# kasvii/GATOR

Hardware: AMD Instinct MI355X
Metric: meshes/sec (B=256, J=17) GATOR forward (higher is better)
Workload: dtype f32; 1 GPU; B=256 synthetic Human3.6M 17-joint poses per GPU, GAT+MDR forward fp32; batch_per_gpu=256, global_batch=256, num_joint=17, impl=fused, parallelism=dp1, mode=gather

## Files before the change

gator_amd/csrc/forward_plan.h:

```cpp
#pragma once
#include <cstddef>

#ifdef __HIP__
#define GATOR_PLAN_HD __host__ __device__
#else
#define GATOR_PLAN_HD
#endif

namespace gator {

constexpr int kVT = 14;
constexpr int kMdrCtrChunks = 64;
constexpr int kTiledTokens = 128;

struct FusedOptions {
    bool gat_x3 = true;
    bool gat8 = true;
    bool gat8_h4 = true;
    bool gat8_lobyte = true;
    bool gat8_tail = true;
    bool gat_tiled_h4 = true;
    int gat_tiled = -1;
    int gat_tiled_min_batch = 1024;
    int mdr_x3 = 2;
    int up_x3 = 2;
    int mdr_persist = -1;
    int mdr_persist_chunk = 0;
    int mdr_persist_grid = 0;
    bool mdr_head_partials = true;
    bool c3_mdr = true;
    bool c3_encoder = true;
    bool c3_up_w1 = true;
    bool c3_up_bf16 = false;
    bool c3_guard = true;
    bool graph = false;
    int subbatch_streams = 0;
    int gat8_dbg = 0;
    bool gat_stamps = false;
    int mdr_cut = 0;
    bool mdr_stamps = false;
    bool mdr_solo = false;
    bool mdr_ends = false;
};

constexpr int kCtrError = 8, kCtrDone = 32;
struct MdrChunkPlan {
    int nch, base, rem;
    GATOR_PLAN_HD void locate(int b, int& ch, int& b0, int& n) const {
        const int split = rem * (base + 1);
        if (b < split) { ch = b / (base + 1); n = base + 1; b0 = ch * n; }
        else { ch = rem + (b - split) / base; n = base; b0 = split + (ch - rem) * base; }
    }
    GATOR_PLAN_HD size_t block(int ch) const {
        const int big = ch < rem ? ch : rem;
        return (size_t)ch * kCtrDone + 4 * ((size_t)big * (base + 1) + (size_t)(ch - big) * base);
    }
};
inline bool operator==(const MdrChunkPlan& a, const MdrChunkPlan& b) { return a.nch == b.nch && a.base == b.base && a.rem == b.rem; }

struct Gat8Form { bool h4; int lr; bool h2, lb, tail; };
struct GatForm { bool x3k, tail; };
struct TiledForm { int J; bool h4, h2; };
inline bool operator==(const Gat8Form& a, const Gat8Form& b) { return a.h4 == b.h4 && a.lr == b.lr && a.h2 == b.h2 && a.lb == b.lb && a.tail == b.tail; }
inline bool operator==(const GatForm& a, const GatForm& b) { return a.x3k == b.x3k && a.tail == b.tail; }
inline bool operator==(const TiledForm& a, const TiledForm& b) { return a.J == b.J && a.h4 == b.h4 && a.h2 == b.h2; }
enum class PlanEntry { FORWARD, GAT, MDR };
enum class SampleEncoder { NONE, GAT, GAT8 };
enum class CtrZero { NOBODY, MDR_JOINT, GAT_JOINT, GAT8_TAIL };
enum class MdrHead { FINISH, WHOLE_HOIST, WHOLE };
enum class Regressor { NONE, FP32, X3, X2, BF16 };
struct RegressorPlan { Regressor form; bool with_joints, w1; };

struct ForwardPlan {
    int n_tiled = 0, n_tail = 0;
    SampleEncoder sample = SampleEncoder::NONE;
    TiledForm tiled{0, false, false};
    Gat8Form gat8{false, 0, false, false, false};
    GatForm gat{false, false};
    bool enc16 = false, fused_tail = false;
    CtrZero ctr_zero = CtrZero::NOBODY;
    int xa = -1, grid = 0; bool persist = false;
    MdrChunkPlan chunks{1, 0, 0};
    MdrHead head = MdrHead::FINISH; RegressorPlan up{Regressor::NONE, false, false};
};
inline bool operator==(const ForwardPlan& a, const ForwardPlan& b) {
    return a.n_tiled == b.n_tiled && a.n_tail == b.n_tail && a.sample == b.sample && a.tiled == b.tiled && a.gat8 == b.gat8 && a.gat == b.gat && a.enc16 == b.enc16 &&
           a.fused_tail == b.fused_tail && a.ctr_zero == b.ctr_zero && a.xa == b.xa && a.grid == b.grid && a.persist == b.persist && a.chunks == b.chunks &&
           a.head == b.head && a.up.form == b.up.form && a.up.with_joints == b.up.with_joints && a.up.w1 == b.up.w1;
}

inline int plan_tiled_samples(const FusedOptions& o, int J, int n_cu, int B, int pin) {
    if (!o.gat_x3 || pin == 0) return 0;
    if (pin == 1) return B;
    if (B < o.gat_tiled_min_batch) return 0;
    const int round = n_cu * (kTiledTokens / J), n_tiled = (B / round) * round;
    return B - n_tiled > 4 * n_cu ? B : n_tiled;
}

inline RegressorPlan plan_regressor(const FusedOptions& o, bool bf16, bool with_joints) {
    const Regressor form = bf16 && o.c3_up_bf16 ? Regressor::BF16 : o.up_x3 == 0 ? Regressor::FP32 : o.up_x3 == 2 ? Regressor::X2 : Regressor::X3;
    return RegressorPlan{form, with_joints, form == Regressor::X2 && bf16 && o.c3_up_w1};
}

inline bool plan_mdr_persist(const FusedOptions& o, int n_cu, int B) {
    if (o.mdr_stamps) return false;
    if (o.mdr_persist >= 0) return o.mdr_persist > 0;
    return n_cu == 256 && (B * kVT + 3) / 4 >= 3 * n_cu;
}

inline MdrChunkPlan plan_mdr_chunks(const FusedOptions& o, int xa, int B) {
    int nch = o.mdr_persist_chunk > 0 ? (B + o.mdr_persist_chunk - 1) / o.mdr_persist_chunk : (xa == 3 ? (B + 383) / 384 : B / 256);
    nch = nch < 1 ? 1 : nch > kMdrCtrChunks ? kMdrCtrChunks : nch;
    return MdrChunkPlan{nch, B / nch, B % nch};
}

inline const char* plan_forward(const FusedOptions& o, int J, int n_cu, int B, PlanEntry entry, bool bf16, bool with_joints, int pin, ForwardPlan* out) {
    ForwardPlan p;
    if (with_joints && (o.up_x3 == 0 || bf16)) return "gator_forward_joints_f32 needs the split-precision vertex regressor";
    if (entry == PlanEntry::GAT) {
        p.sample = SampleEncoder::GAT; p.gat = GatForm{o.gat_x3, true};
        *out = p;
        return nullptr;
    }
    if (entry == PlanEntry::FORWARD) {
        p.n_tiled = plan_tiled_samples(o, J, n_cu, B, pin);
        p.enc16 = bf16 && o.c3_encoder;
        if (p.n_tiled > 0 && p.enc16 && !o.gat_tiled_h4) return "the 16-bit encoder needs the four-product weight image (GATOR_GAT_TILED_H4=1, the default)";
        if (p.n_tiled > 0) p.tiled = TiledForm{J == 17 ? 17 : 19, o.gat_tiled_h4, p.enc16};
        if (p.n_tiled < B && !o.gat8) {
            p.sample = SampleEncoder::GAT; p.gat = GatForm{o.gat_x3, false};
        } else if (p.n_tiled < B) {
            p.sample = SampleEncoder::GAT8;
            if (p.enc16 && !o.gat8_h4) return "the 16-bit encoder needs the four-product weight stream (GATOR_GAT8_H4=1, the default)";
            if (J > 20) return "k_gat8: more than 20 joints (gator_create admits 17 and 19)";
            const bool lb = o.gat8_lobyte && !p.enc16;
            p.fused_tail = o.gat8_tail && (p.enc16 || o.gat8_lobyte);
            if (p.fused_tail && !(o.gat8_h4 && (p.enc16 || lb))) return "k_gat8: no fused tail on the three-plane weight stream";
            p.gat8 = o.gat8_h4 ? Gat8Form{true, J <= 18 ? 10 : 12, p.enc16, lb, p.fused_tail} : Gat8Form{false, 16, false, false, false};
        }
        p.n_tail = p.fused_tail ? p.n_tiled : B;
    }
    if (o.mdr_persist != 0) p.ctr_zero = entry == PlanEntry::MDR ? CtrZero::MDR_JOINT : p.fused_tail ? CtrZero::GAT8_TAIL : CtrZero::GAT_JOINT;
    const bool half16 = bf16 && o.c3_mdr;
    if (half16 && o.mdr_x3 != 2) return "16-bit MDR layers need GATOR_MDR_X3=2 (the default)";
    p.xa = half16 ? 3 : o.mdr_x3;
    p.persist = plan_mdr_persist(o, n_cu, B);
    p.grid = !p.persist ? 0 : o.mdr_persist_grid > 0 ? o.mdr_persist_grid : 2 * n_cu;
    p.chunks = p.persist ? plan_mdr_chunks(o, p.xa, B) : MdrChunkPlan{1, B, 0};
    p.head = o.mdr_head_partials ? MdrHead::FINISH : B <= 2 * n_cu ? MdrHead::WHOLE_HOIST : MdrHead::WHOLE;
    p.up = plan_regressor(o, bf16, with_joints);
    *out = p;
    return nullptr;
}

}
```

gator_amd/csrc/fused_api.hip:

```cpp
#include <hip/hip_runtime.h>

#include <algorithm>
#include <cmath>
#include <cstdlib>
#include <type_traits>
#include <vector>

#include "fused_state.h"
#include "x3_common.h"

namespace gator {
namespace {

static void graph_slot_free(FusedState::GraphSlot& g) {
    if (g.exec) (void)hipGraphExecDestroy((hipGraphExec_t)g.exec);
    if (g.graph) (void)hipGraphDestroy((hipGraph_t)g.graph);
    g.exec = g.graph = nullptr;
}
static void graphs_clear(FusedState* f) {
    for (auto& g : f->graphs) graph_slot_free(g);
    f->graphs.clear();
}
int fused_ensure_ws(gator_ctx* c, FusedWs& w, int B) {
    FusedState* f = c->fused;
    if (w.base && B <= w.cap) return GATOR_OK;
    if (w.base) {
        GATOR_HIP_CHECK(hipDeviceSynchronize());
        graphs_clear(f);
    }
    const int cap = B, MT = (cap + 31) / 32, J = c->J;
    const size_t tiles = (size_t)cap * kVT * 2 * kTile;
    size_t n = 0;
    auto layout = [&](float* block) {
        n = 0;
        auto region = [&](auto*& member, size_t floats) {
            if (block) member = reinterpret_cast<std::remove_reference_t<decltype(member)>>(block + n);
            n += (floats + 63) & ~(size_t)63;
        };
        region(w.vcp, (size_t)MT * 3 * kCB * kTile); region(w.vc, (size_t)cap * kV * 3);
        region(w.vf, 3 * tiles); region(w.q, 9 * tiles / 2); region(w.k, 9 * tiles / 2); region(w.v, 9 * tiles / 2);
        region(w.jkv, (size_t)cap * 12 * kTile); region(w.hf, (size_t)cap * kV * 32); region(w.lbf, (size_t)cap * kV * kE);
        region(w.feat, (size_t)cap * J * kC); region(w.vcp3, std::max(upsample_x3_vcp_elems(cap), upsample_x2_vcp_elems(cap)) / 2);
        region(w.lpart, gat_tail_part_floats(cap, J)); region(w.mdr_ctr, mdr_ctr_words(cap)); region(w.hpart, (size_t)cap * kVT * 128);
    };
    layout(nullptr);
    GATOR_TRY(w.base.alloc(n * sizeof(float)));
    GATOR_HIP_CHECK(hipMemset(w.base, 0, n * sizeof(float)));
    GATOR_HIP_CHECK(hipDeviceSynchronize());
    w.cap = cap;
    layout(w.base);
    return GATOR_OK;
}

std::vector<float> d2h(const float* p, size_t n) {
    std::vector<float> v(n);
    (void)hipMemcpy(v.data(), p, n * sizeof(float), hipMemcpyDeviceToHost);
    return v;
}

template <class F>
void fill_tile(float* dst, F tab) {
    for (int g = 0; g < 4; ++g)
        for (int lane = 0; lane < 64; ++lane)
            for (int j = 0; j < 4; ++j) dst[(g * 64 + lane) * 4 + j] = tab(lane & 31, 8 * g + 4 * (lane >> 5) + j);
}

int read_fused_options(const gator_ctx* c, FusedOptions* o) {
    auto flag = [](const char* name, bool dflt) { const char* e = getenv(name); return e ? atoi(e) != 0 : dflt; };
    auto num = [](const char* name, int dflt) { const char* e = getenv(name); return e ? atoi(e) : dflt; };
    auto set = [](const char* name) { return getenv(name) != nullptr; };
    const bool exact = c->arithmetic == GATOR_ARITH_EXACT_SPLIT;
    o->gat_x3 = flag("GATOR_GAT_X3", true);
    o->gat8 = o->gat_x3 && flag("GATOR_GAT8", true);
    o->gat8_h4 = !exact && flag("GATOR_GAT8_H4", true);
    o->gat8_lobyte = o->gat8 && o->gat8_h4 && flag("GATOR_GAT8_LOBYTE", true);
    o->gat_tiled_h4 = !exact && flag("GATOR_GAT_TILED_H4", true);
    o->gat_tiled = num("GATOR_GAT_TILED", -1);
    if (const int m = num("GATOR_GAT_TILED_MIN_BATCH", 0); m > 0) o->gat_tiled_min_batch = m;
    o->mdr_x3 = exact ? 1 : num("GATOR_MDR_X3", 2);
    o->up_x3 = exact ? 1 : num("GATOR_UPSAMPLE_X3", 2);
    if (c->parts & GATOR_PART_MDR) {
        if (o->up_x3 < 0 || o->up_x3 > 2) return fail(GATOR_EINVAL, "GATOR_UPSAMPLE_X3 must be 0, 1 or 2");
        if (o->mdr_x3 < 0 || o->mdr_x3 > 2) return fail(GATOR_EINVAL, "GATOR_MDR_X3 must be 0, 1 or 2");
    }
    o->gat8_tail = o->gat8 && o->gat8_h4 && o->mdr_x3 == 2 && flag("GATOR_GAT8_TAIL", true);
    o->mdr_persist = set("GATOR_MDR_PERSIST") ? flag("GATOR_MDR_PERSIST", false) : -1;
    o->mdr_persist_chunk = num("GATOR_MDR_PERSIST_CHUNK", 0);
    o->mdr_persist_grid = num("GATOR_MDR_PERSIST_GRID", 0);
    o->mdr_head_partials = flag("GATOR_MDR_HEAD_PARTIALS", true);
    o->c3_mdr = o->mdr_x3 == 2 && flag("GATOR_C3_MDR", true);
    o->c3_encoder = o->gat8 && o->gat8_h4 && o->gat_tiled_h4 && flag("GATOR_C3_ENCODER", true);
    o->c3_up_w1 = flag("GATOR_C3_UPSAMPLE_W1", true);
    o->c3_up_bf16 = o->up_x3 != 2 || flag("GATOR_C3_UPSAMPLE_BF16", false);
    o->c3_guard = flag("GATOR_C3_GUARD", true);
    o->graph = flag("GATOR_GRAPH", false);
    o->subbatch_streams = num("GATOR_SUBBATCH_STREAMS", 0);
#ifdef GATOR_DIAG
    o->gat8_dbg = num("GATOR_GAT8_DBG", 0);
    o->gat_stamps = set("GATOR_GAT_STAMPS");
    o->mdr_cut = num("GATOR_MDR_CUT", 0);
    o->mdr_stamps = set("GATOR_MDR_STAMPS");
    o->mdr_solo = set("GATOR_MDR_SOLO");
    o->mdr_ends = set("GATOR_MDR_ENDS");
#endif
    return GATOR_OK;
}

static double sym_eig_max(std::vector<double>& A, int n) {
    for (int sweep = 0; sweep < 64; ++sweep) {
        double off = 0, all = 0;
        for (int p = 0; p < n; ++p)
            for (int q = 0; q < n; ++q) { all += A[p * n + q] * A[p * n + q]; if (q > p) off += A[p * n + q] * A[p * n + q]; }
        if (!(off > 1e-30 * all)) break;
        for (int p = 0; p < n; ++p)
            for (int q = p + 1; q < n; ++q) {
                const double apq = A[p * n + q];
                if (apq == 0) continue;
                const double th = (A[q * n + q] - A[p * n + p]) / (2 * apq);
                const double t = (th >= 0 ? 1.0 : -1.0) / (std::fabs(th) + std::sqrt(th * th + 1));
                const double cs = 1 / std::sqrt(t * t + 1), sn = t * cs;
                for (int k = 0; k < n; ++k) {
                    const double kp = A[k * n + p], kq = A[k * n + q];
                    A[k * n + p] = cs * kp - sn * kq; A[k * n + q] = sn * kp + cs * kq;
                }
                for (int k = 0; k < n; ++k) {
                    const double pk = A[p * n + k], qk = A[q * n + k];
                    A[p * n + k] = cs * pk - sn * qk; A[q * n + k] = sn * pk + cs * qk;
                }
            }
    }
    double m = 0;
    for (int i = 0; i < n; ++i) m = std::max(m, A[i * n + i]);
    return m;
}

static double sigma_max_rows(const std::vector<float>& W, int r0, int n, int K) {
    std::vector<double> G((size_t)n * n);
    for (int i = 0; i < n; ++i)
        for (int j = 0; j < n; ++j) {
            double acc = 0;
            for (int k = 0; k < K; ++k) acc += (double)W[(size_t)(r0 + i) * K + k] * (double)W[(size_t)(r0 + j) * K + k];
            G[i * n + j] = acc;
        }
    return std::sqrt(std::max(sym_eig_max(G, n), 0.0));
}
static double norm_rows(const std::vector<float>& v, int r0, int n) {
    double s = 0;
    for (int i = 0; i < n; ++i) s += (double)v[r0 + i] * v[r0 + i];
    return std::sqrt(s);
}
static double max_abs(const std::vector<float>& v) {
    double m = 0;
    for (float x : v) m = std::max(m, (double)std::fabs(x));
    return m;
}

float c3_logit_bound(const Weights& w, const float* hop_bias, int J) {
    double worst = 0;
    for (int li = 0; li < 3; ++li) {
        const MdrLayerW& r = w.lay[li];
        const std::vector<float> wq = d2h(r.sa_w[0], 64 * 64), wk = d2h(r.sa_w[1], 64 * 64), bq = d2h(r.sa_b[0], 64), bk = d2h(r.sa_b[1], 64),
                                 a2 = d2h(r.a2, 64), b2 = d2h(r.b2, 64);
        const double xn = max_abs(a2) * std::sqrt(63.0) + norm_rows(b2, 0, 64);
        for (int hd = 0; hd < 2; ++hd)
            worst = std::max(worst, (sigma_max_rows(wq, 32 * hd, 32, 64) * xn + norm_rows(bq, 32 * hd, 32)) *
                                        (sigma_max_rows(wk, 32 * hd, 32, 64) * xn + norm_rows(bk, 32 * hd, 32)) / std::sqrt(32.0));
        const std::vector<float> cq = d2h(r.wq, 64 * 64), ck = d2h(r.wk, 64 * 64), n1w = d2h(r.n1w, 64), n1b = d2h(r.n1b, 64);
// ... 232 lines not shown
                if (rc) return rc;
                if (!h3_set_holds(ratio)) h3_demote(f, GATOR_H3SET_MDR);
            }
            if (f->opt.mdr_x3 != 2) rc = fused_repack_x3(f->lay[0].wq, f->wxbuf, ntiles, stream);
            if (rc) return rc;
        }
        float* hbd = take(64);
        GATOR_HIP_CHECK(hipMemcpy(hbd, hb.data(), 32 * sizeof(float), hipMemcpyHostToDevice));
        f->head_b = hbd;
    }
    {
        float* dst = take(10 * kTile);
        int rc = fused_pack_linear(w.jfeat_w, 133, 1, 64, 133, dst, stream);
        if (rc) return rc;
        f->jfeat_p = dst;
        float* d128 = take(8 * kTile);
        rc = fused_pack_linear(w.jfeat_w + 5, 133, 1, 64, 128, d128, stream);
        if (rc) return rc;
        f->jfeat128_p = d128;
        if (f->opt.mdr_x3 == 2) {
            float& ratio = f->h3_tile_ratio[GATOR_H3SET_JFEAT];
            GATOR_TRY(f->jf128_h3.alloc((size_t)8 * kTileX3 * sizeof(float)));
            rc = fused_repack_h3(d128, f->jf128_h3, 8, &f->jf128_wshift, &ratio, stream);
            if (rc) return rc;
            if (!h3_set_holds(ratio)) { f->jf128_h3.reset(); h3_demote(f, GATOR_H3SET_JFEAT); }
        }
        const std::vector<float> jw = d2h(w.jfeat_w, 64 * 133);
        std::vector<float> j5(5 * 64);
        for (int i = 0; i < 5; ++i)
            for (int n = 0; n < 64; ++n) j5[i * 64 + n] = jw[n * 133 + i];
        float* j5d = take(kTile);
        GATOR_HIP_CHECK(hipMemcpy(j5d, j5.data(), j5.size() * sizeof(float), hipMemcpyHostToDevice));
        f->jfeat5 = j5d;
        const std::vector<float> pj = d2h(w.pos_j, (size_t)(c->J + 1) * 64);
        std::vector<float> pt(2 * kTile);
        for (int nb = 0; nb < 2; ++nb)
            fill_tile(pt.data() + (size_t)nb * kTile, [&](int t, int ch) { return t < c->J ? pj[(size_t)(t + 1) * 64 + 32 * nb + ch] : 0.f; });
        float* pd = take(2 * kTile);
        GATOR_HIP_CHECK(hipMemcpy(pd, pt.data(), pt.size() * sizeof(float), hipMemcpyHostToDevice));
        f->posj_T = pd;
    }
    {
        const std::vector<float> vw = d2h(w.vfeat_w, 64 * 6), vb = d2h(w.vfeat_b, 64), pv = d2h(w.pos_v, (size_t)(kV + 1) * 64), v4 = d2h(w.v431, kV * 3);
        std::vector<float> base((size_t)kVT * 2 * kTile, 0.f), w3(3 * 64);
        for (int t = 0; t < kVT; ++t)
            for (int nb = 0; nb < 2; ++nb)
                for (int g = 0; g < 4; ++g)
                    for (int lane = 0; lane < 64; ++lane)
                        for (int j = 0; j < 4; ++j) {
                            const int token = 32 * t + (lane & 31), ch = 32 * nb + 8 * g + 4 * (lane >> 5) + j;
                            if (token >= kV) continue;
                            double s = (double)vb[ch];
                            for (int i = 0; i < 3; ++i) s += (double)vw[ch * 6 + i] * (double)v4[token * 3 + i];
                            base[(((size_t)(t * 2 + nb) * 4 + g) * 64 + lane) * 4 + j] = (float)(s + (double)pv[(size_t)(token + 1) * 64 + ch]);
                        }
        for (int i = 0; i < 3; ++i)
            for (int ch = 0; ch < 64; ++ch) w3[i * 64 + ch] = vw[ch * 6 + 3 + i];
        float* bd = take(base.size());
        GATOR_HIP_CHECK(hipMemcpy(bd, base.data(), base.size() * sizeof(float), hipMemcpyHostToDevice));
        f->tok_base = bd;
        float* wd = take(3 * 64);
        GATOR_HIP_CHECK(hipMemcpy(wd, w3.data(), w3.size() * sizeof(float), hipMemcpyHostToDevice));
        f->tok_w3 = wd;
    }
    GATOR_HIP_CHECK(hipStreamSynchronize((hipStream_t)stream));
    return GATOR_OK;
}

FusedState::~FusedState() {
    for (FusedWs& w : sets) { w.base.reset(); w.vcp16.reset(); }
    graphs_clear(this);
    if (cap_stream) (void)hipStreamDestroy((hipStream_t)cap_stream);
    if (aux_stream) (void)hipStreamDestroy((hipStream_t)aux_stream);
    if (ev_fork) (void)hipEventDestroy((hipEvent_t)ev_fork);
    if (ev_join) (void)hipEventDestroy((hipEvent_t)ev_join);
}

void fused_destroy(gator_ctx* c) {
    delete c->fused;
    c->fused = nullptr;
}

int launch_upsample_any(const FusedState* f, const gator_ctx* c, const FusedWs& ws, const RegressorPlan& r, int B, float* verts, void* stream) {
    return r.form == Regressor::FP32 ? launch_upsample(f, c, ws, B, verts, stream) : r.form == Regressor::X2 ? launch_upsample_x2(f, c, ws, B, verts, stream, r.with_joints, r.w1) : launch_upsample_x3(f, c, ws, B, verts, stream, r.with_joints);
}

static int fused_plan(const gator_ctx* c, int B, PlanEntry entry, bool bf16, bool with_joints, ForwardPlan* p) {
    const FusedState* f = c->fused;
    const char* why = plan_forward(f->opt, c->J, f->n_cu, B, entry, bf16, with_joints, f->gat_tiled, p);
    return why ? fail(GATOR_EUNSUPPORTED, "%s", why) : GATOR_OK;
}

int fused_gat_forward(gator_ctx* c, const float* pose2d, int B, float* x_out, float* feat, void* stream) {
    ForwardPlan p;
    GATOR_TRY(fused_plan(c, B, PlanEntry::GAT, false, false, &p));
    StageTimer tm(c, "gat", stream);
    return launch_gat(c, c->fused, p.gat, pose2d, B, x_out, feat, stream, B, 0);
}

int fused_upsample(gator_ctx* c, const float* vert431, int B, float* verts, void* stream) {
    FusedState* f = c->fused;
    FusedWs& ws = f->sets[0];
    GATOR_TRY(fused_ensure_ws(c, ws, B));
    const RegressorPlan r = plan_regressor(f->opt, false, false);
    int rc = r.form == Regressor::FP32 ? launch_pack_vc(vert431, B, ws.vcp, stream)
         : r.form == Regressor::X2 ? launch_pack_vc_x2(vert431, B, ws.vcp3, stream) : launch_pack_vc_x3(vert431, B, ws.cap, ws.vcp3, stream);
    if (rc) return rc;
    StageTimer tm(c, "upsample", stream);
    return launch_upsample_any(f, c, ws, r, B, verts, stream);
}

static int fused_upsample_bf16_in(gator_ctx* c, FusedWs& ws, const float* vert431, int B, float* verts, void* stream) {
    GATOR_TRY(fused_ensure_ws(c, ws, B));
    FusedState* f = c->fused;
    if (!f->up_w16) {
        GATOR_TRY(f->up_w16.alloc(upsample_bf16_weight_elems() * 2));
        GATOR_TRY(pack_upsample_bf16(c->w.up_w, f->up_w16, stream));
        GATOR_HIP_CHECK(hipStreamSynchronize((hipStream_t)stream));
    }
    if (B > ws.vcp16_cap) {
        if (ws.vcp16) GATOR_HIP_CHECK(hipDeviceSynchronize());
        GATOR_TRY(ws.vcp16.alloc(upsample_bf16_vcp_elems(B) * 2));
        ws.vcp16_cap = B;
    }
    StageTimer tm(c, "upsample_bf16", stream);
    return launch_upsample_bf16(f, c, ws, vert431, B, verts, stream);
}

int fused_upsample_bf16(gator_ctx* c, const float* vert431, int B, float* verts, void* stream) {
    return fused_upsample_bf16_in(c, c->fused->sets[0], vert431, B, verts, stream);
}

static int fused_regress(gator_ctx* c, FusedWs& ws, const RegressorPlan& r, int B, float* verts, void* stream) {
    if (r.form == Regressor::BF16) return fused_upsample_bf16_in(c, ws, ws.vc, B, verts, stream);
    StageTimer tm(c, "upsample", stream);
    return launch_upsample_any(c->fused, c, ws, r, B, verts, stream);
}

int fused_mdr_forward(gator_ctx* c, const float* pc, int B, float* verts, void* stream) {
    FusedWs& ws = c->fused->sets[0];
    ForwardPlan p;
    GATOR_TRY(fused_plan(c, B, PlanEntry::MDR, false, false, &p));
    GATOR_TRY(fused_ensure_ws(c, ws, B));
    GATOR_TRY(launch_mdr(c, c->fused, ws, p, pc, B, stream, nullptr, nullptr));
    return fused_regress(c, ws, p.up, B, verts, stream);
}

static int fused_forward_one(gator_ctx* c, FusedWs& ws, const ForwardPlan& p, const float* pose2d, int B, float* verts, float* pose3d, void* stream, float* joints);

int fused_set_graph_replay(gator_ctx* c, int on) {
    FusedState* f = c->fused;
    if (!f) return fail(GATOR_EUNSUPPORTED, "gator_set_graph_replay: fused ctx only");
    if (on >= 0) {
        if (!on && f->graph_replay) { GATOR_HIP_CHECK(hipDeviceSynchronize()); graphs_clear(f); }
        f->graph_replay = on != 0;
    }
    return (int)std::min<unsigned long long>(f->graph_launches, 0x7fffffffull);
}

static int fused_forward_graph(gator_ctx* c, FusedWs& ws, const ForwardPlan& p, const float* pose2d, int B, float* verts, float* pose3d, void* stream) {
    FusedState* f = c->fused;
    int rc = fused_ensure_ws(c, ws, B);
    if (rc) return rc;
    FusedState::GraphSlot* slot = nullptr;
    for (auto& g : f->graphs)
        if (g.B == B && g.in == pose2d && g.verts == verts && g.pose3d == pose3d && g.ws == ws.base.get() && g.plan == p) { slot = &g; break; }
    if (!slot) {
        if ((int)f->graphs.size() >= FusedState::kGraphSlots) {
            auto lru = std::min_element(f->graphs.begin(), f->graphs.end(), [](const FusedState::GraphSlot& a, const FusedState::GraphSlot& b) {
                return (a.exec != nullptr) != (b.exec != nullptr) ? a.exec == nullptr : a.used < b.used; });
            if (lru->exec) GATOR_HIP_CHECK(hipDeviceSynchronize());
            graph_slot_free(*lru);
            f->graphs.erase(lru);
        }
        FusedState::GraphSlot g;
        g.B = B; g.in = pose2d; g.verts = verts; g.pose3d = pose3d; g.plan = p; g.ws = ws.base.get();
        g.used = ++f->graph_clock;
        f->graphs.push_back(g);
        return fused_forward_one(c, ws, p, pose2d, B, verts, pose3d, stream, nullptr);
    }
    slot->used = ++f->graph_clock;
    if (!slot->exec) {
        if (!f->cap_stream) {
            hipStream_t s2;
            GATOR_HIP_CHECK(hipStreamCreateWithFlags(&s2, hipStreamNonBlocking));
            f->cap_stream = s2;
        }
// ... 174 lines not shown
```

gator_amd/csrc/fused_state.h:

```cpp
#pragma once
#include "internal.h"
#include "forward_plan.h"
#include <vector>

namespace gator {

constexpr int kOB = 216;
constexpr int kCB = 14;
constexpr int kTile = 32 * 32;
__host__ __device__ inline size_t mdr_ctr_words(int B) { return (size_t)32 * kMdrCtrChunks + (size_t)4 * B; }

struct MdrLayerP {
    const float *wq, *wk, *wv, *proj, *fc1, *fc2, *sa[4];
};

enum { V_N1W = 0, V_N1B = 128, V_QKVB = 256, V_PROJB = 640, V_GCNB = 768, V_LIN0B = 896, V_BACKB = 1024, V_N2W = 1152,
       V_N2B = 1280, V_FC1B = 1408, V_FC2B = 1920, V_TOTAL = 2048 };

struct GatBlockPk {
    const float *qkv, *proj, *w0, *w1, *lin0, *lin1, *back, *fc1, *fc2;
    const float *mc, *mdT, *aoffT, *f1b;
};

struct FusedWs {
// ... 35 lines not shown
    DevBuf<float> jf128_h3;
    int jf128_wshift = 0;
    int mdr_wshift = 0;
    float h3_tile_ratio[4] = {0.f, 0.f, 0.f, 0.f};
    int h3_demoted = 0;
    float c3_logit_bound = 0.f;
    DevBuf<void> up_w2;
    float up_w2_unscale = 1.f;
    DevBuf<void> up_w16;
    DevBuf<void> jr_blk, jr_ent;
    DevBuf<float> jr_w;
    DevBuf<int> jr_rowptr;
    DevBuf<float> jr_P;
    int jr_nnz = 0, jr_nj = 0, jr_cap = 0;
    DevBuf<float> blk_tap;
    int blk_tap_cap = 0;
    MdrLayerP lay[3];
    const float* head_w = nullptr;
    const float* head_b = nullptr;
    const float* tok_base = nullptr;
    const float* tok_w3 = nullptr;
    struct GraphSlot {
        int B = 0; const void *in = nullptr, *verts = nullptr, *pose3d = nullptr;
        ForwardPlan plan; const void* ws = nullptr;
        void *graph = nullptr, *exec = nullptr;
        unsigned long long used = 0;
    };
    static constexpr int kGraphSlots = 8;
    bool graph_replay = false;
    void* cap_stream = nullptr;
    std::vector<GraphSlot> graphs;
    unsigned long long graph_clock = 0, graph_launches = 0;
    FusedWs sets[2];
    void* aux_stream = nullptr;
    void *ev_fork = nullptr, *ev_join = nullptr;
    const float* jfeat_p = nullptr;
    const float* jfeat5 = nullptr;
    const float* jfeat128_p = nullptr;
    const float* posj_T = nullptr;
};

inline void h3_demote(FusedState* f, int set) {
    FusedOptions& o = f->opt;
    f->h3_demoted |= 1 << set;
    if (set == GATOR_H3SET_GAT8) o.gat8_h4 = false;
    if (set == GATOR_H3SET_GAT_TILED) o.gat_tiled_h4 = false;
    if (set == GATOR_H3SET_MDR) o.mdr_x3 = 1;
    if (set == GATOR_H3SET_JFEAT) o.gat8_tail = false;
    o.gat8_lobyte = o.gat8_lobyte && o.gat8_h4;
    o.gat8_tail = o.gat8_tail && o.gat8_h4 && o.mdr_x3 == 2;
    o.c3_mdr = o.c3_mdr && o.mdr_x3 == 2;
    o.c3_encoder = o.c3_encoder && o.gat8_h4 && o.gat_tiled_h4;
}

int fused_pack_linear(const float* W, int64_t wsn, int64_t wsk, int N, int K, float* dst, void* stream);
inline int nblk32(int n) { return (n + 31) / 32; }
int launch_pack_vc(const float* vc, int B, float* vcp, void* stream);
int launch_upsample(const FusedState* f, const gator_ctx* c, const FusedWs& ws, int B, float* verts, void* stream);
int gat_prepare_device();
int gat_ensure_blk_tap(gator_ctx* c, FusedState* f, int B);
int launch_gat(gator_ctx* c, FusedState* f, const GatForm& form, const float* pose2d, int B, float* x_out, float* feat, void* stream, int B_total, int tap_row0);
int gat8_build_stream(FusedState* f, void* stream);
int gat8_prepare_device();
int launch_gat8(gator_ctx* c, FusedState* f, FusedWs& ws, const ForwardPlan& p, const float* pose2d, int B, float* pose3d, void* stream);
int gat_tiled_prepare_device();
int launch_gat_tiled(gator_ctx* c, FusedState* f, FusedWs& ws, const ForwardPlan& p, const float* pose2d, int B, void* stream);
size_t gat_tail_part_floats(int B, int J);
int launch_gat_tail(gator_ctx* c, FusedState* f, FusedWs& ws, const ForwardPlan& p, const float* pose2d, float* x_out, void* stream);
size_t upsample_bf16_weight_elems();
size_t upsample_bf16_vcp_elems(int B);
int pack_upsample_bf16(const float* up_w, void* dst, void* stream);
int launch_upsample_bf16(const FusedState* f, const gator_ctx* c, const FusedWs& ws, const float* vc, int B, float* verts, void* stream);
size_t upsample_x3_weight_elems();
size_t upsample_x3_vcp_elems(int B);
int pack_upsample_x3(const float* up_w, void* dst, void* stream);
int launch_pack_vc_x3(const float* vc, int B, int cap, void* vcp3, void* stream);
int launch_upsample_x3(const FusedState* f, const gator_ctx* c, const FusedWs& ws, int B, float* verts, void* stream, bool with_joints);
int launch_jreg_reduce(const FusedState* f, int B, float* joints, void* stream);
size_t upsample_x2_weight_elems();
size_t upsample_x2_vcp_elems(int B);
int upsample_x2_prepare_device();
int pack_upsample_x2(const float* up_w, void* dst, float* unscale, void* stream);
int launch_pack_vc_x2(const float* vc, int B, void* vcp2, void* stream);
int launch_upsample_x2(const FusedState* f, const gator_ctx* c, const FusedWs& ws, int B, float* verts, void* stream, bool with_joints, bool w1);
int launch_upsample_any(const FusedState* f, const gator_ctx* c, const FusedWs& ws, const RegressorPlan& r, int B, float* verts, void* stream);
int launch_mdr(gator_ctx* c, FusedState* f, FusedWs& ws, const ForwardPlan& p, const float* pc, int B, void* stream, const float* x_out, const float* pose2d);
int launch_mdr_joint(gator_ctx* c, FusedState* f, FusedWs& ws, const ForwardPlan& p, const float* pc, int B, void* stream);
int launch_mdr_head(gator_ctx* c, FusedState* f, FusedWs& ws, const ForwardPlan& p, int B, void* stream, const float* pose2d);

}
```

gator_amd/csrc/upsample_x2.hip:

```cpp
#include <cmath>
#include <cstring>

#include "upsample_common.h"

namespace gator {
namespace {

constexpr int kNBuf = 4, kStageFrags = 36;
constexpr int kActShift = 4;

__device__ __forceinline__ void split2(float x, _Float16& h, _Float16& l) {
    h = (_Float16)x;
    l = (_Float16)(x - (float)h);
}

__global__ void k_pack_up_x2(const float* __restrict__ w, _Float16* __restrict__ dst, int64_t n_frag_pairs, float scale) {
    const int64_t e = (int64_t)blockIdx.x * blockDim.x + threadIdx.x;
    if (e >= n_frag_pairs * 512) return;
    const int j = e & 7, lane = (e >> 3) & 63;
    int64_t r = e >> 9;
    const int tap = r % 3; r /= 3;
    const int o2 = r & 1; r >>= 1;
    const int s = r % kS16;
    const int op = (int)(r / kS16);
    const int o = 32 * (2 * op + o2) + (lane & 31), c = 16 * s + 8 * (lane >> 5) + j;
    const float x = (o < kNV && c < kV) ? w[((int64_t)o * kV + c) * 3 + tap] * scale : 0.f;
    _Float16 h, l;
    split2(x, h, l);
    const int64_t pair = (((int64_t)op * kS16 + s) * 2 + o2) * 3 + tap;
    dst[(pair * 2 + 0) * 512 + lane * 8 + j] = h;
    dst[(pair * 2 + 1) * 512 + lane * 8 + j] = l;
}
__global__ void k_pack_vc_x2(const float* __restrict__ vc, int B, _Float16* __restrict__ ap, int64_t n_frag_pairs) {
    const int64_t e = (int64_t)blockIdx.x * blockDim.x + threadIdx.x;
    if (e >= n_frag_pairs * 512) return;
    const int j = e & 7, lane = (e >> 3) & 63;
    int64_t r = e >> 9;
    const int lp = r % 3; r /= 3;
    const int mi = r & 3; r >>= 2;
    const int s = r % kS16;
    const int mg = (int)(r / kS16);
    const int smp = 32 * (4 * mg + mi) + (lane & 31), c = 16 * s + 8 * (lane >> 5) + j;
    const float x = (smp < B && c < kV) ? vc[((int64_t)smp * kV + c) * 3 + lp] * (float)(1 << kActShift) : 0.f;
    _Float16 h, l;
    split2(x, h, l);
    const int64_t pair = (((int64_t)mg * kS16 + s) * 4 + mi) * 3 + lp;
    ap[(pair * 2 + 0) * 512 + lane * 8 + j] = h;
    ap[(pair * 2 + 1) * 512 + lane * 8 + j] = l;
}

__global__ void k_absmax(const float* __restrict__ w, int64_t n, unsigned* __restrict__ out) {
    float m = 0.f;
    for (int64_t i = (int64_t)blockIdx.x * blockDim.x + threadIdx.x; i < n; i += (int64_t)gridDim.x * blockDim.x) {
        const float a = fabsf(w[i]);
        m = a > m || a != a ? a : m;
    }
    for (int o = 32; o > 0; o >>= 1) {
        const float q = __shfl_xor(m, o);
        m = q > m || q != q ? q : m;
    }
    if ((threadIdx.x & 63) == 0) atomicMax(out, __float_as_uint(m));
}

__device__ __forceinline__ void dma_frag(const void* base, unsigned lane_off, unsigned lds_dst) {
    unsigned keep;
    asm volatile("s_mov_b32 %0, m0\n\ts_mov_b32 m0, %3\n\ts_nop 0\n\tglobal_load_lds_dwordx4 %1, %2\n\ts_mov_b32 m0, %0"
                 : "=&s"(keep) : "v"(lane_off), "s"(base), "s"(lds_dst) : "memory");
}
template <int N> __device__ __forceinline__ void wait_vm() { asm volatile("s_waitcnt vmcnt(%0)" ::"n"(N) : "memory"); }

template <bool WLO = true>
__global__ __launch_bounds__(512, 1) void k_upsample_x2(const _Float16* __restrict__ ap, const _Float16* __restrict__ wp,
                                                        const float* __restrict__ bias, const float* __restrict__ tpl,
                                                        float* __restrict__ out, int B, int MT, int MG, int nwg, float unscale,
                                                        const JregEpi jr) {
    extern __shared__ __attribute__((aligned(16))) unsigned char lds_raw[];
    f16x8 (*st)[kStageFrags][64] = reinterpret_cast<f16x8 (*)[kStageFrags][64]>(lds_raw);
    const int lane = threadIdx.x & 63, wave = __builtin_amdgcn_readfirstlane(threadIdx.x >> 6);
    const int wg = xcd_remap(blockIdx.x, nwg);
    const int obp = wg / MG, mg = wg % MG;
    const int mi = wave & 3, oi = wave >> 2;
    const int ob = 2 * obp + oi, mt = 4 * mg + mi;
    const bool live = mt < MT;
    const unsigned lane_off = lane * 16;
    const unsigned lds0 = (unsigned)(unsigned long long)lds_raw;
    const char* a_src = reinterpret_cast<const char*>(ap) + (size_t)mg * kS16 * 24 * 1024;
    const char* w_src = reinterpret_cast<const char*>(wp) + (size_t)obp * kS16 * 12 * 1024;
    const char* src[5];
    unsigned stride[5], dsto[5];
#pragma unroll
    for (int i = 0; i < 5; ++i) {
        const int f = wave + 8 * i;
        src[i] = f < 24 ? a_src + f * 1024 : w_src + (f - 24) * 1024;
        stride[i] = f < 24 ? 24 * 1024 : 12 * 1024;
        dsto[i] = lds0 + f * 1024;
    }
    auto issue = [&](int s) {
        const unsigned dst = (unsigned)(s & (kNBuf - 1)) * kStageFrags * 1024;
#pragma unroll
        for (int i = 0; i < 4; ++i) dma_frag(src[i] + (size_t)s * stride[i], lane_off, dst + dsto[i]);
        if (wave < 4) dma_frag(src[4] + (size_t)s * stride[4], lane_off, dst + dsto[4]);
    };
    auto wait_landed = [&](int younger) {
        if (younger >= 1) { if (wave < 4) wait_vm<5>(); else wait_vm<4>(); }
        else wait_vm<0>();
    };
    f32x16 big[3], sm[3], tot[3];
#pragma unroll
    for (int l = 0; l < 3; ++l) { big[l] = zero16(); sm[l] = zero16(); tot[l] = zero16(); }
    f16x8 a[3][2], w[3][2];
    auto load_first = [&](int s) {
        const f16x8 (*cur)[64] = st[s & (kNBuf - 1)];
#pragma unroll
        for (int p = 0; p < 2; ++p) {
            a[0][p] = cur[mi * 6 + p][lane];
            w[0][p] = cur[24 + oi * 6 + p][lane];
            w[1][p] = cur[24 + oi * 6 + 2 + p][lane];
        }
    };
    auto load_rest = [&](int s) {
        const f16x8 (*cur)[64] = st[s & (kNBuf - 1)];
#pragma unroll
        for (int p = 0; p < 2; ++p) {
            a[1][p] = cur[mi * 6 + 2 + p][lane];
            w[2][p] = cur[24 + oi * 6 + 4 + p][lane];
            a[2][p] = cur[mi * 6 + 4 + p][lane];
        }
    };
    issue(0); issue(1); issue(2);
    if (wave < 4) wait_vm<10>(); else wait_vm<8>();
    __builtin_amdgcn_s_barrier();
    load_first(0);
#pragma unroll 1
    for (int s = 0; s < kS16; ++s) {
        if (s + 1 < kS16) wait_landed(kS16 - 2 - s);
        __builtin_amdgcn_s_barrier();
        if (s + 3 < kS16) issue(s + 3);
        load_rest(s);
        if (live) {
#pragma unroll
            for (int lp = 0; lp < 3; ++lp)
#pragma unroll
                for (int k = 2; k >= 0; --k) {
                    const int l = lp + 1 - k;
                    if (l < 0 || l > 2) continue;
                    big[l] = GATOR_MFMA_F16(a[lp][0], w[k][0], big[l]);
                    if constexpr (WLO) sm[l] = GATOR_MFMA_F16(a[lp][0], w[k][1], sm[l]);
                    sm[l] = GATOR_MFMA_F16(a[lp][1], w[k][0], sm[l]);
                }
            if (s % 7 == 6) {
#pragma unroll
                for (int l = 0; l < 3; ++l) { tot[l] += big[l]; big[l] = zero16(); }
            }
        }
        if (s + 1 < kS16) load_first(s + 1);
    }
    const int ov = 32 * ob + (lane & 31), h = lane >> 5;
    if (ov >= kNV || !live) return;
    const float bo = bias[ov];
    const float t0 = tpl[ov * 3], t1 = tpl[ov * 3 + 1], t2 = tpl[ov * 3 + 2];
    const int2 jb = jr.P ? jr.blk[ob] : int2{0, 0};
#pragma unroll
    for (int r = 0; r < 16; ++r) {
        const int smp = 32 * mt + kap(r) + 4 * h;
        if (smp < B) {
            F3 v;
            v.x = ((tot[0][r] + sm[0][r]) * unscale + bo) + t0;
            v.y = ((tot[1][r] + sm[1][r]) * unscale + bo) + t1;
            v.z = ((tot[2][r] + sm[2][r]) * unscale + bo) + t2;
            if (out) *reinterpret_cast<F3*>(out + ((int64_t)smp * kNV + ov) * 3) = v;
            for (int e = jb.x; e < jb.x + jb.y; ++e) {
                const int2 en = jr.ent[e];
                if (en.x == ov) {
                    const float we = jr.w[e];
                    F3 q;
                    q.x = we * v.x; q.y = we * v.y; q.z = we * v.z;
                    *reinterpret_cast<F3*>(jr.P + ((int64_t)smp * jr.nnz + en.y) * 3) = q;
                }
            }
        }
    }
}

constexpr size_t kX2Lds = (size_t)kNBuf * kStageFrags * 1024;

}

size_t upsample_x2_weight_elems() { return (size_t)(kOB / 2) * kS16 * 12 * 512; }
size_t upsample_x2_vcp_elems(int B) { return (size_t)((B + 127) / 128) * kS16 * 24 * 512; }

int upsample_x2_prepare_device() {
    GATOR_HIP_CHECK(hipFuncSetAttribute((const void*)k_upsample_x2<true>, hipFuncAttributeMaxDynamicSharedMemorySize, (int)kX2Lds));
    GATOR_HIP_CHECK(hipFuncSetAttribute((const void*)k_upsample_x2<false>, hipFuncAttributeMaxDynamicSharedMemorySize, (int)kX2Lds));
    return GATOR_OK;
}

int pack_upsample_x2(const float* up_w, void* dst, float* unscale, void* stream) {
    hipStream_t st = (hipStream_t)stream;
    DevBuf<unsigned> d_max;
    GATOR_TRY(d_max.alloc(sizeof(unsigned)));
    GATOR_HIP_CHECK(hipMemsetAsync(d_max, 0, sizeof(unsigned), st));
    const int64_t n = (int64_t)kNV * kV * 3;
    k_absmax<<<1024, 256, 0, st>>>(up_w, n, d_max.get());
    unsigned bits = 0;
    GATOR_HIP_CHECK(hipMemcpyAsync(&bits, d_max, sizeof(unsigned), hipMemcpyDeviceToHost, st));
    GATOR_HIP_CHECK(hipStreamSynchronize(st));
    d_max.reset();
    float wmax;
    static_assert(sizeof(wmax) == sizeof(bits), "float bits");
    memcpy(&wmax, &bits, sizeof(wmax));
    int shift = 0;
    if (wmax > 0.f && std::isfinite(wmax)) {
        int e;
        (void)std::frexp(wmax, &e);
        shift = 14 - e;
        if (shift > 118) shift = 118;
        if (shift < -118) shift = -118;
    }
    const int64_t pairs = (int64_t)upsample_x2_weight_elems() / 1024;
    k_pack_up_x2<<<(unsigned)((pairs * 512 + 255) / 256), 256, 0, st>>>(up_w, (_Float16*)dst, pairs, std::ldexp(1.0f, shift));
    GATOR_HIP_CHECK(hipGetLastError());
    *unscale = std::ldexp(1.0f, -(shift + kActShift));
    return GATOR_OK;
}

int launch_pack_vc_x2(const float* vc, int B, void* vcp2, void* stream) {
    const int64_t pairs = (int64_t)upsample_x2_vcp_elems(B) / 1024;
    k_pack_vc_x2<<<(unsigned)((pairs * 512 + 255) / 256), 256, 0, (hipStream_t)stream>>>(vc, B, (_Float16*)vcp2, pairs);
    GATOR_HIP_CHECK(hipGetLastError());
    return GATOR_OK;
}

int launch_upsample_x2(const FusedState* f, const gator_ctx* c, const FusedWs& ws, int B, float* verts, void* stream, bool with_joints, bool w1) {
    const int MT = (B + 31) / 32, MG = (MT + 3) / 4;
    const JregEpi jr = jreg_epi(f, with_joints);
    const int nwg = (kOB / 2) * MG;
    if (w1) k_upsample_x2<false><<<nwg, 512, kX2Lds, (hipStream_t)stream>>>((const _Float16*)ws.vcp3, (const _Float16*)f->up_w2.get(), c->w.up_b, c->w.v6890,
                                                                           verts, B, MT, MG, nwg, f->up_w2_unscale, jr);
    else k_upsample_x2<true><<<nwg, 512, kX2Lds, (hipStream_t)stream>>>((const _Float16*)ws.vcp3, (const _Float16*)f->up_w2.get(), c->w.up_b, c->w.v6890,
                                                                       verts, B, MT, MG, nwg, f->up_w2_unscale, jr);
    GATOR_HIP_CHECK(hipGetLastError());
    return GATOR_OK;
}

}
```

Measured before the change: 441,400 meshes/sec.

## Add split-role two-ring DMA pipeline to x2 vertex regressor and trim final stage

Adds a second staging scheme for the fp16 x2 upsample kernel. Some waves stream activation fragments into a 3-deep ring while the rest stream weight fragments into a 6-deep ring, with only the live M tiles copied. It is chosen for batches of 64 or fewer, or forced with GATOR_UPSAMPLE_RING=2. The default ring=1 path keeps the old single ring but runs one K stage fewer (kS16-1) and adds a final accumulator flush, which presumes the last K stage is padding. The kernel is now templated on the pipe mode and dispatched through a function-pointer table.

```diff
diff --git a/gator_amd/csrc/forward_plan.h b/gator_amd/csrc/forward_plan.h
--- a/gator_amd/csrc/forward_plan.h
+++ b/gator_amd/csrc/forward_plan.h
@@ -24,6 +24,7 @@
     int gat_tiled_min_batch = 1024;
     int mdr_x3 = 2;
     int up_x3 = 2;
+    int up_ring = 1;
     int mdr_persist = -1;
     int mdr_persist_chunk = 0;
     int mdr_persist_grid = 0;
@@ -69,7 +70,7 @@
 enum class CtrZero { NOBODY, MDR_JOINT, GAT_JOINT, GAT8_TAIL };
 enum class MdrHead { FINISH, WHOLE_HOIST, WHOLE };
 enum class Regressor { NONE, FP32, X3, X2, BF16 };
-struct RegressorPlan { Regressor form; bool with_joints, w1; };
+struct RegressorPlan { Regressor form; bool with_joints, w1; int pipe; };
 
 struct ForwardPlan {
     int n_tiled = 0, n_tail = 0;
@@ -81,12 +82,12 @@
     CtrZero ctr_zero = CtrZero::NOBODY;
     int xa = -1, grid = 0; bool persist = false;
     MdrChunkPlan chunks{1, 0, 0};
-    MdrHead head = MdrHead::FINISH; RegressorPlan up{Regressor::NONE, false, false};
+    MdrHead head = MdrHead::FINISH; RegressorPlan up{Regressor::NONE, false, false, 0};
 };
 inline bool operator==(const ForwardPlan& a, const ForwardPlan& b) {
     return a.n_tiled == b.n_tiled && a.n_tail == b.n_tail && a.sample == b.sample && a.tiled == b.tiled && a.gat8 == b.gat8 && a.gat == b.gat && a.enc16 == b.enc16 &&
            a.fused_tail == b.fused_tail && a.ctr_zero == b.ctr_zero && a.xa == b.xa && a.grid == b.grid && a.persist == b.persist && a.chunks == b.chunks &&
-           a.head == b.head && a.up.form == b.up.form && a.up.with_joints == b.up.with_joints && a.up.w1 == b.up.w1;
+           a.head == b.head && a.up.form == b.up.form && a.up.with_joints == b.up.with_joints && a.up.w1 == b.up.w1 && a.up.pipe == b.up.pipe;
 }
 
 inline int plan_tiled_samples(const FusedOptions& o, int J, int n_cu, int B, int pin) {
@@ -97,9 +98,11 @@
     return B - n_tiled > 4 * n_cu ? B : n_tiled;
 }
 
-inline RegressorPlan plan_regressor(const FusedOptions& o, bool bf16, bool with_joints) {
+constexpr int kTwoRingMaxBatch = 64;
+inline RegressorPlan plan_regressor(const FusedOptions& o, bool bf16, bool with_joints, int B) {
     const Regressor form = bf16 && o.c3_up_bf16 ? Regressor::BF16 : o.up_x3 == 0 ? Regressor::FP32 : o.up_x3 == 2 ? Regressor::X2 : Regressor::X3;
-    return RegressorPlan{form, with_joints, form == Regressor::X2 && bf16 && o.c3_up_w1};
+    const int pipe = form != Regressor::X2 || o.up_ring == 0 ? 0 : o.up_ring == 2 || B <= kTwoRingMaxBatch ? 2 : 1;
+    return RegressorPlan{form, with_joints, form == Regressor::X2 && bf16 && o.c3_up_w1, pipe};
 }
 
 inline bool plan_mdr_persist(const FusedOptions& o, int n_cu, int B) {
@@ -148,7 +151,7 @@
     p.grid = !p.persist ? 0 : o.mdr_persist_grid > 0 ? o.mdr_persist_grid : 2 * n_cu;
     p.chunks = p.persist ? plan_mdr_chunks(o, p.xa, B) : MdrChunkPlan{1, B, 0};
     p.head = o.mdr_head_partials ? MdrHead::FINISH : B <= 2 * n_cu ? MdrHead::WHOLE_HOIST : MdrHead::WHOLE;
-    p.up = plan_regressor(o, bf16, with_joints);
+    p.up = plan_regressor(o, bf16, with_joints, B);
     *out = p;
     return nullptr;
 }
diff --git a/gator_amd/csrc/fused_api.hip b/gator_amd/csrc/fused_api.hip
--- a/gator_amd/csrc/fused_api.hip
+++ b/gator_amd/csrc/fused_api.hip
@@ -83,6 +83,8 @@
         if (o->up_x3 < 0 || o->up_x3 > 2) return fail(GATOR_EINVAL, "GATOR_UPSAMPLE_X3 must be 0, 1 or 2");
         if (o->mdr_x3 < 0 || o->mdr_x3 > 2) return fail(GATOR_EINVAL, "GATOR_MDR_X3 must be 0, 1 or 2");
     }
+    o->up_ring = num("GATOR_UPSAMPLE_RING", 1);
+    if ((c->parts & GATOR_PART_MDR) && (o->up_ring < 0 || o->up_ring > 2)) return fail(GATOR_EINVAL, "GATOR_UPSAMPLE_RING must be 0, 1 or 2");
     o->gat8_tail = o->gat8 && o->gat8_h4 && o->mdr_x3 == 2 && flag("GATOR_GAT8_TAIL", true);
     o->mdr_persist = set("GATOR_MDR_PERSIST") ? flag("GATOR_MDR_PERSIST", false) : -1;
     o->mdr_persist_chunk = num("GATOR_MDR_PERSIST_CHUNK", 0);
@@ -481,7 +483,7 @@
 }
 
 int launch_upsample_any(const FusedState* f, const gator_ctx* c, const FusedWs& ws, const RegressorPlan& r, int B, float* verts, void* stream) {
-    return r.form == Regressor::FP32 ? launch_upsample(f, c, ws, B, verts, stream) : r.form == Regressor::X2 ? launch_upsample_x2(f, c, ws, B, verts, stream, r.with_joints, r.w1) : launch_upsample_x3(f, c, ws, B, verts, stream, r.with_joints);
+    return r.form == Regressor::FP32 ? launch_upsample(f, c, ws, B, verts, stream) : r.form == Regressor::X2 ? launch_upsample_x2(f, c, ws, B, verts, stream, r.with_joints, r.w1, r.pipe) : launch_upsample_x3(f, c, ws, B, verts, stream, r.with_joints);
 }
 
 static int fused_plan(const gator_ctx* c, int B, PlanEntry entry, bool bf16, bool with_joints, ForwardPlan* p) {
@@ -501,7 +503,7 @@
     FusedState* f = c->fused;
     FusedWs& ws = f->sets[0];
     GATOR_TRY(fused_ensure_ws(c, ws, B));
-    const RegressorPlan r = plan_regressor(f->opt, false, false);
+    const RegressorPlan r = plan_regressor(f->opt, false, false, B);
     int rc = r.form == Regressor::FP32 ? launch_pack_vc(vert431, B, ws.vcp, stream)
          : r.form == Regressor::X2 ? launch_pack_vc_x2(vert431, B, ws.vcp3, stream) : launch_pack_vc_x3(vert431, B, ws.cap, ws.vcp3, stream);
     if (rc) return rc;
diff --git a/gator_amd/csrc/fused_state.h b/gator_amd/csrc/fused_state.h
--- a/gator_amd/csrc/fused_state.h
+++ b/gator_amd/csrc/fused_state.h
@@ -141,7 +141,7 @@
 int upsample_x2_prepare_device();
 int pack_upsample_x2(const float* up_w, void* dst, float* unscale, void* stream);
 int launch_pack_vc_x2(const float* vc, int B, void* vcp2, void* stream);
-int launch_upsample_x2(const FusedState* f, const gator_ctx* c, const FusedWs& ws, int B, float* verts, void* stream, bool with_joints, bool w1);
+int launch_upsample_x2(const FusedState* f, const gator_ctx* c, const FusedWs& ws, int B, float* verts, void* stream, bool with_joints, bool w1, int pipe);
 int launch_upsample_any(const FusedState* f, const gator_ctx* c, const FusedWs& ws, const RegressorPlan& r, int B, float* verts, void* stream);
 int launch_mdr(gator_ctx* c, FusedState* f, FusedWs& ws, const ForwardPlan& p, const float* pc, int B, void* stream, const float* x_out, const float* pose2d);
 int launch_mdr_joint(gator_ctx* c, FusedState* f, FusedWs& ws, const ForwardPlan& p, const float* pc, int B, void* stream);
diff --git a/gator_amd/csrc/upsample_x2.hip b/gator_amd/csrc/upsample_x2.hip
--- a/gator_amd/csrc/upsample_x2.hip
+++ b/gator_amd/csrc/upsample_x2.hip
@@ -69,13 +69,25 @@
 }
 template <int N> __device__ __forceinline__ void wait_vm() { asm volatile("s_waitcnt vmcnt(%0)" ::"n"(N) : "memory"); }
 
-template <bool WLO = true>
+constexpr int kRingAct = 3, kRingW = 6;
+constexpr int kRingActWaves = 6;
+constexpr size_t kX2Lds = (size_t)kNBuf * kStageFrags * 1024;
+static_assert((size_t)(kRingAct * 24 + kRingW * 12) * 1024 == kX2Lds, "the two rings fill the one ring's LDS");
+
+__device__ __forceinline__ void wait_vm_n(int n) {
+    switch (n) {
+        case 1: wait_vm<1>(); break;   case 2: wait_vm<2>(); break;   case 3: wait_vm<3>(); break;   case 4: wait_vm<4>(); break;
+        case 6: wait_vm<6>(); break;   case 12: wait_vm<12>(); break; case 24: wait_vm<24>(); break; default: wait_vm<0>(); break;
+    }
+}
+
+template <bool WLO = true, int PIPE = 1>
 __global__ __launch_bounds__(512, 1) void k_upsample_x2(const _Float16* __restrict__ ap, const _Float16* __restrict__ wp,
                                                         const float* __restrict__ bias, const float* __restrict__ tpl,
                                                         float* __restrict__ out, int B, int MT, int MG, int nwg, float unscale,
                                                         const JregEpi jr) {
     extern __shared__ __attribute__((aligned(16))) unsigned char lds_raw[];
-    f16x8 (*st)[kStageFrags][64] = reinterpret_cast<f16x8 (*)[kStageFrags][64]>(lds_raw);
+    const f16x8 (*frag)[64] = reinterpret_cast<const f16x8 (*)[64]>(lds_raw);
     const int lane = threadIdx.x & 63, wave = __builtin_amdgcn_readfirstlane(threadIdx.x >> 6);
     const int wg = xcd_remap(blockIdx.x, nwg);
     const int obp = wg / MG, mg = wg % MG;
@@ -86,74 +98,121 @@
     const unsigned lds0 = (unsigned)(unsigned long long)lds_raw;
     const char* a_src = reinterpret_cast<const char*>(ap) + (size_t)mg * kS16 * 24 * 1024;
     const char* w_src = reinterpret_cast<const char*>(wp) + (size_t)obp * kS16 * 12 * 1024;
-    const char* src[5];
-    unsigned stride[5], dsto[5];
-#pragma unroll
-    for (int i = 0; i < 5; ++i) {
-        const int f = wave + 8 * i;
-        src[i] = f < 24 ? a_src + f * 1024 : w_src + (f - 24) * 1024;
-        stride[i] = f < 24 ? 24 * 1024 : 12 * 1024;
-        dsto[i] = lds0 + f * 1024;
-    }
-    auto issue = [&](int s) {
-        const unsigned dst = (unsigned)(s & (kNBuf - 1)) * kStageFrags * 1024;
-#pragma unroll
-        for (int i = 0; i < 4; ++i) dma_frag(src[i] + (size_t)s * stride[i], lane_off, dst + dsto[i]);
-        if (wave < 4) dma_frag(src[4] + (size_t)s * stride[4], lane_off, dst + dsto[4]);
-    };
-    auto wait_landed = [&](int younger) {
-        if (younger >= 1) { if (wave < 4) wait_vm<5>(); else wait_vm<4>(); }
-        else wait_vm<0>();
-    };
     f32x16 big[3], sm[3], tot[3];
 #pragma unroll
     for (int l = 0; l < 3; ++l) { big[l] = zero16(); sm[l] = zero16(); tot[l] = zero16(); }
     f16x8 a[3][2], w[3][2];
-    auto load_first = [&](int s) {
-        const f16x8 (*cur)[64] = st[s & (kNBuf - 1)];
+    auto load_first = [&](int fa, int fw) {
 #pragma unroll
         for (int p = 0; p < 2; ++p) {
-            a[0][p] = cur[mi * 6 + p][lane];
-            w[0][p] = cur[24 + oi * 6 + p][lane];
-            w[1][p] = cur[24 + oi * 6 + 2 + p][lane];
+            a[0][p] = frag[fa + p][lane];
+            w[0][p] = frag[fw + p][lane];
+            w[1][p] = frag[fw + 2 + p][lane];
         }
     };
-    auto load_rest = [&](int s) {
-        const f16x8 (*cur)[64] = st[s & (kNBuf - 1)];
+    auto load_rest = [&](int fa, int fw) {
 #pragma unroll
         for (int p = 0; p < 2; ++p) {
-            a[1][p] = cur[mi * 6 + 2 + p][lane];
-            w[2][p] = cur[24 + oi * 6 + 4 + p][lane];
-            a[2][p] = cur[mi * 6 + 4 + p][lane];
+            a[1][p] = frag[fa + 2 + p][lane];
+            w[2][p] = frag[fw + 4 + p][lane];
+            a[2][p] = frag[fa + 4 + p][lane];
         }
     };
-    issue(0); issue(1); issue(2);
-    if (wave < 4) wait_vm<10>(); else wait_vm<8>();
-    __builtin_amdgcn_s_barrier();
-    load_first(0);
+    auto flush = [&]() {
+#pragma unroll
+        for (int l = 0; l < 3; ++l) { tot[l] += big[l]; big[l] = zero16(); }
+    };
+    auto products = [&](int s) {
+#pragma unroll
+        for (int lp = 0; lp < 3; ++lp)
+#pragma unroll
+            for (int k = 2; k >= 0; --k) {
+                const int l = lp + 1 - k;
+                if (l < 0 || l > 2) continue;
+                big[l] = GATOR_MFMA_F16(a[lp][0], w[k][0], big[l]);
+                if constexpr (WLO) sm[l] = GATOR_MFMA_F16(a[lp][0], w[k][1], sm[l]);
+                sm[l] = GATOR_MFMA_F16(a[lp][1], w[k][0], sm[l]);
+            }
+        if (s % 7 == 6) flush();
+    };
+    if constexpr (PIPE < 2) {
+        constexpr int KS = PIPE == 1 ? kS16 - 1 : kS16;
+        const char* src[5];
+        unsigned stride[5], dsto[5];
+#pragma unroll
+        for (int i = 0; i < 5; ++i) {
+            const int f = wave + 8 * i;
+            src[i] = f < 24 ? a_src + f * 1024 : w_src + (f - 24) * 1024;
+            stride[i] = f < 24 ? 24 * 1024 : 12 * 1024;
+            dsto[i] = lds0 + f * 1024;
+        }
+        auto issue = [&](int s) {
+            const unsigned dst = (unsigned)(s & (kNBuf - 1)) * kStageFrags * 1024;
+#pragma unroll
+            for (int i = 0; i < 4; ++i) dma_frag(src[i] + (size_t)s * stride[i], lane_off, dst + dsto[i]);
+            if (wave < 4) dma_frag(src[4] + (size_t)s * stride[4], lane_off, dst + dsto[4]);
+        };
+        auto wait_landed = [&](int younger) {
+            if (younger >= 1) { if (wave < 4) wait_vm<5>(); else wait_vm<4>(); }
+            else wait_vm<0>();
+        };
+        auto fa = [&](int s) { return (s & (kNBuf - 1)) * kStageFrags + mi * 6; };
+        auto fw = [&](int s) { return (s & (kNBuf - 1)) * kStageFrags + 24 + oi * 6; };
+        issue(0); issue(1); issue(2);
+        if (wave < 4) wait_vm<10>(); else wait_vm<8>();
+        __builtin_amdgcn_s_barrier();
+        load_first(fa(0), fw(0));
 #pragma unroll 1
-    for (int s = 0; s < kS16; ++s) {
-        if (s + 1 < kS16) wait_landed(kS16 - 2 - s);
+        for (int s = 0; s < KS; ++s) {
+            if (s + 1 < KS) wait_landed(KS - 2 - s);
+            __builtin_amdgcn_s_barrier();
+            if (s + 3 < KS) issue(s + 3);
+            load_rest(fa(s), fw(s));
+            if (live) products(s);
+            if (s + 1 < KS) load_first(fa(s + 1), fw(s + 1));
+        }
+        if (PIPE == 1 && live) flush();
+    } else {
+        constexpr int NA = kRingAct, NW = kRingW, KS = kS16 - 1;
+        static_assert(NA == 3, "the activation role waits for everything it issued: one stage in flight");
+        const bool copies_act = wave < kRingActWaves;
+        const int n_live = MT - 4 * mg < 4 ? MT - 4 * mg : 4;
+        const int N = copies_act ? NA : NW, per_stage = copies_act ? n_live : 6;
+        auto issue = [&](int s) {
+            if (copies_act) {
+                const char* src = a_src + (size_t)s * (24 * 1024) + wave * 1024;
+                const unsigned dst = lds0 + (unsigned)((s % NA) * 24 + wave) * 1024;
+#pragma unroll
+                for (int i = 0; i < 4; ++i)
+                    if (i < n_live) dma_frag(src + i * 6 * 1024, lane_off, dst + i * 6 * 1024);
+            } else {
+                const int f0 = (wave - kRingActWaves) * 6;
+                const char* src = w_src + (size_t)s * (12 * 1024) + f0 * 1024;
+                const unsigned dst = lds0 + (unsigned)(NA * 24 + (s % NW) * 12 + f0) * 1024;
+#pragma unroll
+                for (int j = 0; j < 6; ++j) dma_frag(src + j * 1024, lane_off, dst + j * 1024);
+            }
+        };
+        auto fa = [&](int s) { return (s % NA) * 24 + mi * 6; };
+        auto fw = [&](int s) { return NA * 24 + (s % NW) * 12 + oi * 6; };
+        for (int s = 0; s < N - 1; ++s) issue(s);
+        wait_vm_n((N - 2) * per_stage);
         __builtin_amdgcn_s_barrier();
-        if (s + 3 < kS16) issue(s + 3);
-        load_rest(s);
-        if (live) {
-#pragma unroll
-            for (int lp = 0; lp < 3; ++lp)
-#pragma unroll
-                for (int k = 2; k >= 0; --k) {
-                    const int l = lp + 1 - k;
-                    if (l < 0 || l > 2) continue;
-                    big[l] = GATOR_MFMA_F16(a[lp][0], w[k][0], big[l]);
-                    if constexpr (WLO) sm[l] = GATOR_MFMA_F16(a[lp][0], w[k][1], sm[l]);
-                    sm[l] = GATOR_MFMA_F16(a[lp][1], w[k][0], sm[l]);
-                }
-            if (s % 7 == 6) {
-#pragma unroll
-                for (int l = 0; l < 3; ++l) { tot[l] += big[l]; big[l] = zero16(); }
+        load_first(fa(0), fw(0));
+#pragma unroll 1
+        for (int s = 0; s < KS; ++s) {
+            if (s + N - 2 < KS) {
+                if (copies_act) wait_vm<0>(); else wait_vm<(NW - 3) * 6>();
+            } else if (s + 1 < KS) {
+                wait_vm_n((KS - 2 - s) * per_stage);
             }
-        }
-        if (s + 1 < kS16) load_first(s + 1);
+            __builtin_amdgcn_s_barrier();
+            if (s + N - 1 < KS) issue(s + N - 1);
+            load_rest(fa(s), fw(s));
+            if (live) products(s);
+            if (s + 1 < KS) load_first(fa(s + 1), fw(s + 1));
+        }
+        if (live) flush();
     }
     const int ov = 32 * ob + (lane & 31), h = lane >> 5;
     if (ov >= kNV || !live) return;
@@ -182,7 +241,12 @@
     }
 }
 
-constexpr size_t kX2Lds = (size_t)kNBuf * kStageFrags * 1024;
+using X2Kernel = void (*)(const _Float16*, const _Float16*, const float*, const float*, float*, int, int, int, int, float, const JregEpi);
+X2Kernel x2_kernel(bool w1, int pipe) {
+    static const X2Kernel k[2][3] = {{k_upsample_x2<true, 0>, k_upsample_x2<true, 1>, k_upsample_x2<true, 2>},
+                                     {k_upsample_x2<false, 0>, k_upsample_x2<false, 1>, k_upsample_x2<false, 2>}};
+    return k[w1][pipe];
+}
 
 }
 
@@ -190,8 +254,9 @@
 size_t upsample_x2_vcp_elems(int B) { return (size_t)((B + 127) / 128) * kS16 * 24 * 512; }
 
 int upsample_x2_prepare_device() {
-    GATOR_HIP_CHECK(hipFuncSetAttribute((const void*)k_upsample_x2<true>, hipFuncAttributeMaxDynamicSharedMemorySize, (int)kX2Lds));
-    GATOR_HIP_CHECK(hipFuncSetAttribute((const void*)k_upsample_x2<false>, hipFuncAttributeMaxDynamicSharedMemorySize, (int)kX2Lds));
+    for (int w1 = 0; w1 < 2; ++w1)
+        for (int pipe = 0; pipe < 3; ++pipe)
+            GATOR_HIP_CHECK(hipFuncSetAttribute((const void*)x2_kernel(w1, pipe), hipFuncAttributeMaxDynamicSharedMemorySize, (int)kX2Lds));
     return GATOR_OK;
 }
 
@@ -231,14 +296,12 @@
     return GATOR_OK;
 }
 
-int launch_upsample_x2(const FusedState* f, const gator_ctx* c, const FusedWs& ws, int B, float* verts, void* stream, bool with_joints, bool w1) {
+int launch_upsample_x2(const FusedState* f, const gator_ctx* c, const FusedWs& ws, int B, float* verts, void* stream, bool with_joints, bool w1, int pipe) {
     const int MT = (B + 31) / 32, MG = (MT + 3) / 4;
     const JregEpi jr = jreg_epi(f, with_joints);
     const int nwg = (kOB / 2) * MG;
-    if (w1) k_upsample_x2<false><<<nwg, 512, kX2Lds, (hipStream_t)stream>>>((const _Float16*)ws.vcp3, (const _Float16*)f->up_w2.get(), c->w.up_b, c->w.v6890,
-                                                                           verts, B, MT, MG, nwg, f->up_w2_unscale, jr);
-    else k_upsample_x2<true><<<nwg, 512, kX2Lds, (hipStream_t)stream>>>((const _Float16*)ws.vcp3, (const _Float16*)f->up_w2.get(), c->w.up_b, c->w.v6890,
-                                                                       verts, B, MT, MG, nwg, f->up_w2_unscale, jr);
+    x2_kernel(w1, pipe)<<<nwg, 512, kX2Lds,(hipStream_t)stream>>>((const _Float16*)ws.vcp3, (const _Float16*)f->up_w2.get(), c->w.up_b, c->w.v6890,
+                                                                               verts, B, MT, MG, nwg, f->up_w2_unscale, jr);
     GATOR_HIP_CHECK(hipGetLastError());
     return GATOR_OK;
 }
```

After: 442,600 meshes/sec, median of 6. About the same (+0.3%).
